# dbking77/ar_slam

Hardware: AMD Instinct MI355X
Metric: LM iterations/sec + ms-to-converged reproj-RMS, 10k-capture synthetic graph (higher is better)
Workload: dtype f64

## Files before the change

### ar_slam_amd/csrc/llt_dag.hip

```cpp
#include "llt_tile.h"
#include "llt_wt.h"

#include <algorithm>
#include <climits>
#include <cmath>

namespace arslam {

namespace {

#ifndef ARSLAM_PIPE_FROM
#define ARSLAM_PIPE_FROM 3
#endif
constexpr int kPipeFrom = ARSLAM_PIPE_FROM;
#ifndef ARSLAM_PIPE_W2
#define ARSLAM_PIPE_W2 1
#endif
constexpr int kPipeW2 = ARSLAM_PIPE_W2;

struct DagArgs {
  double *S;
  int T;
  double *Ld;
  double *ltd;
  const int *rec;
  const int2 *ks_tiles;
  const int *ks;
  int *claimed;
  const int2 *waits;
  int *counters;
  int n_tiles;
  int n_tasks;
  double *part;
  int *split_cnt;
  int *flag;
  int t_begin, t_end;
  int *ticket;
  int *progress;
  unsigned long long *trace;
  int first_store;
  int *started;
  int wg_limit;
};

typedef int int16v __attribute__((ext_vector_type(16)));
struct DagRecV {
  int16v a, b;
  __device__ __forceinline__ int operator[](int i) const { return i < 16 ? a[i] : b[i - 16]; }
};
__device__ __forceinline__ DagRecV load_rec(const int *p) {
  DagRecV r;
  asm volatile("s_load_dwordx16 %0, %2, 0x0\n\ts_load_dwordx16 %1, %2, 0x40\n\ts_waitcnt lgkmcnt(0)"
               : "=s"(r.a), "=s"(r.b)
               : "s"(p)
               : "memory");
  return r;
}
__device__ __forceinline__ DagRecV lds_rec(const int *s) {
  DagRecV r;
#pragma unroll
  for (int i = 0; i < 16; ++i) {
    r.a[i] = __builtin_amdgcn_readfirstlane(s[i]);
    r.b[i] = __builtin_amdgcn_readfirstlane(s[16 + i]);
  }
  return r;
}

enum DagShSlot {
  kShTicket = 0,
  kShBad = 1,
  kShRun = 2,
  kShLast = 3,
  kShClaim = 4,
  kShFetchReq = 6,
  kShFoldCnt = 7,
  kShPipe0 = 8,
  kShThirds = 11,
  kShSolveStep0 = 12,
  kShAkkHalf0 = 16,
  kShTake = 18,
  kShContMet0 = 20,
  kShRec = 24,
  kShInts = kShRec + kDagRecInts
};
static_assert(kShThirds == kShPipe0 + kPfCaller && kShPipe0 + kPfFlags <= kShSolveStep0, "the POTRF pipeline's flags");
static_assert(kShContMet0 + 1 < kShRec && kShInts % 2 == 0, "the slots fit before the record; colx stays 8-byte aligned");

#define DAG_PROGRESS(slot, v)                                                                  \
  do {                                                                                         \
    if (a.progress && tid == 0)                                                                \
      __hip_atomic_store(a.progress + kDagProgressInts * blockIdx.x + (slot), (v), __ATOMIC_RELAXED,          \
                         __HIP_MEMORY_SCOPE_SYSTEM);                                            \
  } while (0)

#ifdef ARSLAM_DAG_SUBSTAMPS
#define DAG_SUBSTAMP(word)                                                                      \
  do {                                                                                          \
    if (a.trace && tid == 0) a.trace[kDagTraceWords * (long)t + (word)] = realtime();           \
  } while (0)
#else
#define DAG_SUBSTAMP(word) do {} while (0)
#endif

__global__ __launch_bounds__(256, kDagWorkgroupsPerCu) void k_factor_dag(DagArgs a) {
  __shared__ __attribute__((aligned(16))) double lds[2 * T64 * LQ + T64 + kLtdSize + kShInts / 2 + T64];
  double *D = lds, *X = lds + T64 * LQ, *inv = X + T64 * LQ, *LTd = inv + T64;
  int *sh = reinterpret_cast<int *>(LTd + kLtdSize);
  int *sh_rec = sh + kShRec;
  double *colx = LTd + kLtdSize + kShInts / 2;
  int *ready = a.counters, *applied = a.counters + a.n_tiles, *ticket = a.ticket;
  int *inflight = a.counters + 2 * a.n_tiles + kDagOffInflight;
  if ((int)blockIdx.x >= a.wg_limit) return;
  if (threadIdx.x == 0) __hip_atomic_fetch_add(a.started, 1, __ATOMIC_RELAXED, __HIP_MEMORY_SCOPE_AGENT);
  int *cu_flag = a.counters + 2 * a.n_tiles + kDagOffCuFlags;
  int cu_key = 0;
  {
    unsigned hw, xcc;
    asm volatile("s_getreg_b32 %0, hwreg(HW_REG_HW_ID)" : "=s"(hw));
    asm volatile("s_getreg_b32 %0, hwreg(HW_REG_XCC_ID)" : "=s"(xcc));
    cu_key = (int)(((xcc & 7u) << 8) | ((hw >> 8) & 0xffu));
  }
  int next = -1, prev_k = -1;
  bool next_met = false;
  bool fast_next = false;
  for (;;) {
    int tid = threadIdx.x;
    asm volatile("" : "+v"(tid));
    const int w = tid >> 6, lane = tid & 63;
    const int r0 = (w >> 1) * 32, c0 = (w & 1) * 32;
    const int li = lane & 15, lk = lane >> 4;
    const bool cont = next >= 0;
    if (!cont) {
      if (tid == 0) sh[kShTicket] = a.t_begin + atomicAdd(ticket, 1);
      __syncthreads();
      next = sh[kShTicket];
      __syncthreads();
    }
    const int t = __builtin_amdgcn_readfirstlane(next);
    const int pk = prev_k;
    const bool premet = cont && next_met;
    const bool fast = cont && fast_next;
    next = -1;
    prev_k = -1;
    next_met = false;
    fast_next = false;
    DAG_PROGRESS(kProgTicket, t);
    DAG_PROGRESS(kProgPhase, 1);
    if (t >= a.t_end) break;
    const DagRecV r = cont ? lds_rec(sh_rec) : load_rec(a.rec + (long)t * kDagRecInts);
    const int4 task = make_int4(r[kRecType], r[kRecY], r[kRecZ], r[kRecW]);
    DAG_PROGRESS(kProgType, task.x);
    if (a.trace && tid == 0) { a.trace[kDagTraceWords * (long)t + kTrDraw] = realtime(); a.trace[kDagTraceWords * (long)t + kTrWg] = blockIdx.x; }
    const int2 sub = make_int2(r[kRecSub], r[kRecLate]);
    if (w == 0) {
      int3 unmet;
      bool expired = false;
      const bool ok =
          premet || dag_wait(a.counters, a.waits, r[kRecWait0], sub.y, a.flag, lane, task.x != 2, &unmet, &expired);
      if (lane == 0) {
        if (!ok) dag_fault(a.flag, a.counters, a.n_tiles, ticket, 1, t, unmet, expired);
        sh[kShRun] = (cont || r[kRecMaxdep] < 0 || atomicCAS(a.claimed + t, 0, 1) == 0) ? 1 : 0;
      }
    }
    if (!fast) {
      __syncthreads();
      if (!sh[kShRun]) continue;
    }
    DAG_PROGRESS(kProgPhase, 2);
    if (a.trace && tid == 0) a.trace[kDagTraceWords * (long)t + kTrMet] = realtime();
    if (task.x != 2) __builtin_amdgcn_s_setprio(3);
    if (task.x == 0) {
      const int k = task.y;
      const int c = sub.x >= 0 ? r[kRecCont] : -1;
      const int apf_tile = sub.x >= 0 ? r[kRecContAkk] : -1;
      const bool apf = apf_tile >= 0;
      const double *apf_src = a.S + (long)max(apf_tile, 0) * (T64 * T64);
      bool ap_met = false;
      int c_rec = 0;
      int2 c_wait = make_int2(0, 0);
      dbl2 apv[16];
#pragma unroll
      for (int u = 0; u < 16; ++u) apv[u] = dbl2{0.0, 0.0};
      bool ap_ok = false;
      if (tid == 0)
        __hip_atomic_store(cu_flag + cu_key, 1, __ATOMIC_RELAXED, __HIP_MEMORY_SCOPE_AGENT);
      const int4 fit = make_int4(0, r[kRecQ0], r[kRecQ1], 0);
      const bool akk_in_d = cont && sh[kShAkkHalf0] && sh[kShAkkHalf0 + 1];
      const bool fold_in = task.z >= 0 && fit.z - fit.y == 1;
      if (fold_in) {
        const double *Akk = a.S + (long)task.w * (T64 * T64);
        if (cont && r[kRecFoldK0] == pk) {
          if (!akk_in_d) load_tile_wt(Akk, D, tid);
        } else load_two_tiles_wt(Akk, D, a.S + (long)r[kRecFoldTile0] * (T64 * T64), X, tid);
      } else if (task.z >= 0) {
        const int4 it = fit;
        dbl4 acc[4] = {{0, 0, 0, 0}, {0, 0, 0, 0}, {0, 0, 0, 0}, {0, 0, 0, 0}};
        double akk[16];
        {
          const double *Akk = a.S + (long)task.w * (T64 * T64);
#pragma unroll
          for (int q = 0; q < 4; ++q) {
            const int rb = r0 + (q >> 1) * 16, cb = c0 + (q & 1) * 16;
#pragma unroll
            for (int reg = 0; reg < 4; ++reg) akk[4 * q + reg] = ld_wt(Akk + (rb + lk + 4 * reg) * T64 + cb + li);
          }
        }
        for (int q = it.y; q < it.z; ++q) {
          if (cont && a.ks[q] == pk) {
            gemm64_nt(X, X, tid, acc);
            continue;
          }
          if (q > it.y) __syncthreads();
          load_tile_wt(a.S + (long)a.ks_tiles[q].x * (T64 * T64), D, tid);
          __syncthreads();
          gemm64_nt(D, D, tid, acc);
        }
        __syncthreads();
#pragma unroll
        for (int q = 0; q < 4; ++q) {
          const int rb = r0 + (q >> 1) * 16, cb = c0 + (q & 1) * 16;
#pragma unroll
          for (int reg = 0; reg < 4; ++reg) D[(rb + lk + 4 * reg) * LQ + cb + li] = akk[4 * q + reg] - acc[q][reg];
        }
      } else {
        load_tile_wt(a.S + (long)task.w * (T64 * T64), D, tid);
      }
      if (!fast) __syncthreads();
      if (a.trace && tid == 0) a.trace[kDagTraceWords * (long)t + kTrLoaded] = realtime();
      const double *pf_src = sub.x >= 0 ? a.S + (long)sub.x * (T64 * T64) : nullptr;
      const int pw0 = sub.y, pw1 = r[kRecWait1];
      const int2 pw_wait = (sub.x >= 0 && pw0 + lane < pw1) ? a.waits[pw0 + lane] : make_int2(0, 0);
      if (tid == 0 && !fast) {
        sh[kShFetchReq] = 0;
        sh[kShSolveStep0] = sh[kShSolveStep0 + 1] = sh[kShSolveStep0 + 2] = sh[kShSolveStep0 + 3] = 0;
        sh[kShTake] = 0;
      }
      bool third_done = false;
      int sdone = 0;
      const bool ok = blocked_potrf64_async(D, inv, LTd, sh + kShBad, sh + kShPipe0, tid, colx, [&](int p, int wv, int ln) {
        auto fetch_third = [&]() {
        auto poll = [&]() {
          if (!pf_src || pw1 - pw0 > 64) return false;
          const int q = pw0 + ln;
          const int got = q < pw1 ? ld_acquire_relaxed(a.counters + pw_wait.x) : 0;
          return __builtin_amdgcn_ballot_w64(q < pw1 && got < pw_wait.y) == 0;
        };
        int lnl = ln;
        asm volatile("" : "+v"(lnl));
        if (p == 0) {
          if (wv == 1 && poll() && ln == 0) *as_lds(sh + kShFetchReq) = -1;
          return;
        }
        if (third_done || lds_get(sh + kShThirds) >= 3) return;
        const int req = lds_get(sh + kShFetchReq);
        bool take = req != 0 && req < p;
        if (req == 0) {
          if (p < 3) {
            if (wv == 1 && poll() && ln == 0) *as_lds(sh + kShFetchReq) = p;
          } else {
            if (!pf_src || pw1 - pw0 > 64) {
              take = false;
            } else if (wv == 1) {
              take = poll();
              lds_set(sh + kShTake, take ? 1 : 2);
            } else {
              lds_wait(sh + kShTake, 1);
              take = lds_get(sh + kShTake) == 1;
            }
          }
        }
        if (take) {
          const int e0 = (wv - 1) * 683, e1 = min(wv * 683, 2048);
          const double *p11[11];
          dbl2 v[11];
#pragma unroll
          for (int u = 0; u < 11; ++u) p11[u] = pf_src + 2 * min(e0 + u * 64 + lnl, e1 - 1);
          ld_wt16x11(p11, v);
#pragma unroll
          for (int u = 0; u < 11; ++u) {
            const int e = e0 + u * 64 + ln, r = e >> 5, c2 = (e & 31) * 2;
            if (e < e1) *reinterpret_cast<dbl2 *>(X + r * LQ + c2) = v[u];
          }
          third_done = true;
          lds_add(sh + kShThirds, ln);
        }
        };
        int c_got = 0;
        bool c_mine = false;
        if (p == 3 && c >= 0 && wv >= 2 && r[kRecContLate] - r[kRecContWait0] <= 64) {
          const int q = r[kRecContWait0] + ln;
          c_mine = q < r[kRecContLate] && c_wait.x != sub.x;
          if (c_mine) c_got = ld_acquire_relaxed(a.counters + c_wait.x);
        }
        fetch_third();
        if (c >= 0 && wv >= 2) {
          const int cw0 = r[kRecContWait0], cw1 = r[kRecContLate];
          if (p == 1 && wv == 3 && ln < kDagRecInts) c_rec = a.rec[(long)c * kDagRecInts + ln];
          if (p == 2) {
            if (wv == 3 && ln < kDagRecInts) sh_rec[ln] = c_rec;
            const int q = cw0 + ln;
            if (q < cw1) c_wait = a.waits[q];
          }
          if (p == 3) {
            const bool met = cw1 - cw0 <= 64 && __builtin_amdgcn_ballot_w64(c_mine && c_got < c_wait.y) == 0;
            if (ln == 0) sh[kShContMet0 + wv - 2] = met ? 1 : 0;
            ap_met = met && apf;
          }
        }
        if (p == 3 && third_done && sdone < 3) lds_wait(sh + kShThirds, 3);
        if (kPipeFrom <= 3 && pf_src && p >= kPipeFrom && sdone < p && lds_get(sh + kShThirds) >= 3) {
          __builtin_amdgcn_fence(__ATOMIC_ACQUIRE, "workgroup");
          for (int st = sdone; st < p; ++st) {
            trsm_step(X, D, LTd, wv - 1, st, ln);
            if (wv == kPipeW2) trsm_step(X, D, LTd, 3, st, ln);
          }
          sdone = p;
          if (ln == 0) {
            sh[kShSolveStep0 + wv - 1] = sdone;
            if (wv == kPipeW2) sh[kShSolveStep0 + 3] = sdone;
          }
        }
      }, X, fold_in, sh + kShFoldCnt);
      const bool keep_flag = sub.x >= 0 && sh[kShThirds] >= 3;
      if (tid == 0 && !keep_flag)
        __hip_atomic_store(cu_flag + cu_key, 0, __ATOMIC_RELAXED, __HIP_MEMORY_SCOPE_AGENT);
      if (a.trace && tid == 0) a.trace[kDagTraceWords * (long)t + kTrFactored] = realtime();
      if (!ok && tid == 0) {
        int first = 0;
        while (first < T64 && D[first * LQ + first] > 0.0) ++first;
        atomicCAS(a.flag, 0, 1 + k * T64 + first);
      }
      double *ltd_g = a.ltd + (long)k * kLtdSize;
      store_tile_wt(a.Ld + (long)k * T64 * T64, D, tid, true);
      for (int e = tid; e < kLtdSize / 2; e += 256)
        st_wt16(ltd_g + 2 * e, *reinterpret_cast<const dbl2 *>(LTd + 2 * e));
      dag_release(tid);
      if (tid == 0) __hip_atomic_fetch_add(ready + task.w, 1, __ATOMIC_RELAXED, __HIP_MEMORY_SCOPE_AGENT);
      if (a.trace && tid == 0) a.trace[kDagTraceWords * (long)t + kTrPublished] = realtime();
      if (sub.x >= 0) {
        const bool pref = sh[kShThirds] >= 3;
        if (!pref) {
          if (w == 0) {
            int3 unmet;
            bool expired = false;
            const bool ok2 = dag_wait(a.counters, a.waits, sub.y, r[kRecWait1], a.flag, lane, true, &unmet, &expired);
            if (!ok2 && lane == 0) dag_fault(a.flag, a.counters, a.n_tiles, ticket, 3, t, unmet, expired);
          }
          __syncthreads();
        }
        double *Ct = a.S + (long)sub.x * (T64 * T64);
        int tk_seen = 0, infl_old = 0, started_seen = 0;
        if (c >= 0 && tid == 0) {
          tk_seen = ld_acquire_relaxed(ticket);
          started_seen = ld_acquire_relaxed(a.started);
          infl_old = atomicAdd(inflight, 1);
        }
        if (!pref) load_tile_wt(Ct, X, tid);
        if (ap_met) {
          int t2 = tid - 128;
          asm volatile("" : "+v"(t2));
          ld_wt16x16_issue(apf_src, t2, apv);
          ap_ok = true;
        }
        __syncthreads();
        DAG_SUBSTAMP(kTrSolveTop);
        const int s0 = pref ? sh[kShSolveStep0 + w] : 0;
        for (int st = s0; st < 2; ++st) trsm_step(X, D, LTd, w, st, lane);
        const bool want = c >= 0 && tid == 0 && a.t_begin + tk_seen > r[kRecContMaxdep] && infl_old < started_seen / 2;
#ifdef ARSLAM_DAG_SUBSTAMPS
        if (a.trace && tid == 0) asm volatile("" ::"v"(tk_seen), "v"(started_seen), "v"(infl_old));
#endif
        DAG_SUBSTAMP(kTrWantKnown);
        int cas_old = 1;
        if (want) cas_old = atomicCAS(a.claimed + c, 0, 1);
        for (int st = max(s0, 2); st < 4; ++st) trsm_step(X, D, LTd, w, st, lane);
        store_elems_wt<64, 512>(Ct, X, 512 * w, lane, false);
        if (keep_flag && tid == 0)
          __hip_atomic_store(cu_flag + cu_key, 0, __ATOMIC_RELAXED, __HIP_MEMORY_SCOPE_AGENT);
        __syncthreads();
        DAG_SUBSTAMP(kTrSolved);
        if (w >= 2) {
          if (ap_ok) {
            ld_wt16x16_wait(apv);
            const int t2 = tid - 128;
#pragma unroll
            for (int u = 0; u < 16; ++u) {
              const int e = u * 128 + t2, row = e >> 5, c2 = (e & 31) * 2;
              *reinterpret_cast<dbl2 *>(D + row * LQ + c2) = apv[u];
            }
          }
          if (lane == 0) sh[kShAkkHalf0 + w - 2] = ap_ok ? 1 : 0;
        }
        if (tid == 0) {
          const int claim = want && cas_old == 0 ? c : -1;
          if (c >= 0 && claim < 0) atomicSub(inflight, 1);
          sh[kShClaim] = claim;
        }
        asm volatile("s_waitcnt vmcnt(0)" ::: "memory");
        __syncthreads();
        DAG_SUBSTAMP(kTrAcked);
        if (tid == 0) __hip_atomic_fetch_add(ready + sub.x, 1, __ATOMIC_RELAXED, __HIP_MEMORY_SCOPE_AGENT);
        if (a.trace && tid == 0) {
          a.trace[kDagTraceWords * (long)t + kTrSubPublished] = realtime();
          const unsigned long long fl = (premet ? 1 : 0) | (akk_in_d ? 2 : 0) | (pref ? 4 : 0) |
                                        (sh[kShContMet0] && sh[kShContMet0 + 1] ? 8 : 0) | (sh[kShClaim] >= 0 ? 16 : 0);
          a.trace[kDagTraceWords * (long)t + kTrWg] = blockIdx.x | (fl << 32);
        }
        __syncthreads();
        next = sh[kShClaim];
        next_met = next >= 0 && sh[kShContMet0] && sh[kShContMet0 + 1];
        if (next >= 0) prev_k = k;
      } else if (r[kRecInv] > 0) {
        blocked_trinv64(D, LTd, X, tid);
        __syncthreads();
        double *Xg = a.Ld + ((long)a.T + k) * T64 * T64;
#pragma unroll
        for (int m = 0; m < 16; ++m) {
          const int e = m * 256 + tid, row = e >> 6, col = e & 63;
          Xg[e] = (row >= col) ? X[col * LQ + row] : 0.0;
        }
      }
    } else if (task.x == 3) {
      const int k = task.y;
      load_tiles_ltd_wt(a.Ld + (long)k * T64 * T64, D, nullptr, nullptr, a.ltd + (long)k * kLtdSize, LTd, tid);
      __syncthreads();
      blocked_trinv64(D, LTd, X, tid);
      __syncthreads();
      double *Xg = a.Ld + ((long)a.T + k) * T64 * T64;
#pragma unroll 4
      for (int m = 0; m < 16; ++m) {
        const int e = m * 256 + tid, r = e >> 6, c = e & 63;
        Xg[e] = (r >= c) ? X[c * LQ + r] : 0.0;
      }
    } else if (task.x == 1) {
      const int k = task.z;
      double *Ct = a.S + (long)task.w * (T64 * T64);
      load_tiles_ltd_wt(Ct, X, a.Ld + (long)k * T64 * T64, D, a.ltd + (long)k * kLtdSize, LTd, tid);
      __syncthreads();
      if (a.trace && tid == 0) a.trace[kDagTraceWords * (long)t + kTrLoaded] = realtime();
      blocked_trsm64(X, D, inv, LTd, tid);
      if (a.trace && tid == 0) a.trace[kDagTraceWords * (long)t + kTrFactored] = realtime();
      store_tile_wt(Ct, X, tid, false);
      dag_release(tid);
      if (tid == 0) __hip_atomic_fetch_add(ready + task.w, 1, __ATOMIC_RELAXED, __HIP_MEMORY_SCOPE_AGENT);
    } else {
      const int4 it = make_int4(0, r[kRecQ0], r[kRecQ1], r[kRecSid]);
      const int ti = r[kRecTi], tj = r[kRecTj], sid = it.w;
      dbl4 acc[4] = {{0, 0, 0, 0}, {0, 0, 0, 0}, {0, 0, 0, 0}, {0, 0, 0, 0}};
      double *C = a.S + (long)task.w * (T64 * T64);
      double cv[16];
      bool c_pre = false;
      if (task.z == 0 && task.w >= a.first_store) {
#pragma unroll
        for (int u = 0; u < 16; ++u) cv[u] = 0.0;
        c_pre = true;
      }
      for (int q = it.y; q < it.z; ++q) {
        const int2 kt = q == it.y ? make_int2(r[kRecTile0I], r[kRecTile0J]) : a.ks_tiles[q];
        if (q > it.y) __syncthreads();
        {
          if (tid == 0) {
            for (int spin = 0; spin < 256 &&
                               __hip_atomic_load(cu_flag + cu_key, __ATOMIC_RELAXED, __HIP_MEMORY_SCOPE_AGENT);
                 ++spin)
              __builtin_amdgcn_s_sleep(8);
          }
          __syncthreads();
        }
        if (q == it.y && sid < 0 && tid == 0)
          sh[kShLast] = (task.z == 0 || ld_acquire_relaxed(applied + task.w) >= task.z) ? 1 : 0;
        if (ti != tj)
          load_two_tiles_wt(a.S + (long)kt.x * (T64 * T64), D, a.S + (long)kt.y * (T64 * T64), X, tid);
        else
          load_tile_wt(a.S + (long)kt.x * (T64 * T64), D, tid);
        __syncthreads();
        const bool c_issue = q == it.z - 1 && sid < 0 && sh[kShLast] && !c_pre;
        if (c_issue) {
#pragma unroll
          for (int u = 0; u < 4; ++u) {
            const int rb = r0 + (u >> 1) * 16, cb = c0 + (u & 1) * 16;
#pragma unroll
            for (int reg = 0; reg < 4; ++reg) cv[4 * u + reg] = ld_wt(C + (rb + lk + 4 * reg) * T64 + cb + li);
          }
          c_pre = true;
        }
        gemm64_nt(D, ti != tj ? X : D, tid, acc);
      }
      bool apply = true;
      if (sid >= 0) {
        const int2 sp = make_int2(r[kRecSplitN], r[kRecSplitP]);
        double *mine = a.part + (long)(sp.y + (sid & 255)) * 4096;
#pragma unroll
        for (int q = 0; q < 4; ++q)
#pragma unroll
          for (int reg = 0; reg < 4; ++reg) st_wt(mine + (4 * q + reg) * 256 + tid, acc[q][reg]);
        dag_release(tid);
        if (tid == 0) {
          const int old = __hip_atomic_fetch_add(a.split_cnt + (sid >> 8), 1, __ATOMIC_RELAXED,
                                                 __HIP_MEMORY_SCOPE_AGENT);
          sh[kShLast] = old == sp.x - 1;
        }
        __syncthreads();
        apply = sh[kShLast] != 0;
        if (apply) {
#pragma unroll
          for (int q = 0; q < 4; ++q) acc[q] = dbl4{0, 0, 0, 0};
          for (int c = 0; c < sp.x; ++c) {
            const double *pc = a.part + (long)(sp.y + c) * 4096;
            double v[16];
            const double *p8[16];
#pragma unroll
            for (int u = 0; u < 16; ++u) p8[u] = pc + u * 256 + tid;
            ld_wt8x8(p8, v);
            ld_wt8x8(p8 + 8, v + 8);
#pragma unroll
            for (int q = 0; q < 4; ++q)
#pragma unroll
              for (int reg = 0; reg < 4; ++reg) acc[q][reg] += v[4 * q + reg];
          }
        }
      }
      DAG_PROGRESS(kProgPhase, 3);
      if (apply && !c_pre) {
        if (tid == 0) {
          long spins = 0;
          int seen;
          WaitTimer tm;
          while ((seen = ld_acquire_relaxed(applied + task.w)) < task.z) {
            __builtin_amdgcn_s_sleep(kPollSleep);
            const bool exp = tm.expired(++spins);
            if (exp || (((spins & 255) == 0) && ld_acquire_relaxed(a.flag) < 0)) {
              dag_fault(a.flag, a.counters, a.n_tiles, ticket, 2, t, make_int3(a.n_tiles + task.w, seen, task.z), exp);
              break;
            }
          }
        }
        __syncthreads();
#pragma unroll
        for (int q = 0; q < 4; ++q) {
          const int rb = r0 + (q >> 1) * 16, cb = c0 + (q & 1) * 16;
#pragma unroll
          for (int reg = 0; reg < 4; ++reg) cv[4 * q + reg] = ld_wt(C + (rb + lk + 4 * reg) * T64 + cb + li);
        }
      }
      if (apply) {
#pragma unroll
        for (int q = 0; q < 4; ++q) {
          const int rb = r0 + (q >> 1) * 16, cb = c0 + (q & 1) * 16;
#pragma unroll
          for (int reg = 0; reg < 4; ++reg)
            st_wt(C + (rb + lk + 4 * reg) * T64 + cb + li, cv[4 * q + reg] - acc[q][reg]);
        }
        dag_release(tid);
        if (tid == 0) __hip_atomic_fetch_add(applied + task.w, 1, __ATOMIC_RELAXED, __HIP_MEMORY_SCOPE_AGENT);
      }
    }
    DAG_PROGRESS(kProgPhase, 4);
    if (cont && tid == 0) atomicSub(inflight, 1);
    __builtin_amdgcn_s_setprio(0);
    if (a.trace && tid == 0) a.trace[kDagTraceWords * (long)t + kTrEnd] = realtime();
  }
  {
    const int tid = threadIdx.x;
    DAG_PROGRESS(kProgPhase, 9);
  }
}

__device__ __forceinline__ void bs_issue_lik(const double *__restrict__ S, int tile, int w, int lane,
                                             double (&lv)[16]) {
  const double *Lik = S + (long)tile * (T64 * T64);
#pragma unroll
  for (int m = 0; m < 16; ++m) lv[m] = Lik[(w + 4 * m) * T64 + lane];
}

__global__ __launch_bounds__(256) void k_bsolve_dag(const double *__restrict__ S, const int *__restrict__ tid_map,
                                                    int T, const double *__restrict__ Ld, long nR,
                                                    const int *__restrict__ cols, const int2 *__restrict__ gather,
                                                    const int *__restrict__ gtile, const int *__restrict__ gbeg,
                                                    int ncols, double *yF, int *counters, int *flag) {
  __shared__ double red[4][T64];
  __shared__ double ys[T64];
  enum { kBsTicket, kBsOk, kBsSlots };
  __shared__ int sh[kBsSlots];
  if (*flag) return;
  const int tid = threadIdx.x, w = tid >> 6, lane = tid & 63;
  int *ticket = counters + T;
  const double *Xinv = Ld + (long)T * T64 * T64;
  const long kr = nR / T64;
  for (;;) {
    if (tid == 0) sh[kBsTicket] = atomicAdd(ticket, 1);
    __syncthreads();
    const int b = __builtin_amdgcn_readfirstlane(sh[kBsTicket]);
    if (b >= ncols) break;
    const int k = cols[b];
    const int g0 = gbeg[b], g1 = gbeg[b + 1];
    const long row0 = (long)k * T64;
    const double *X = Xinv + (long)k * T64 * T64;
    double xv[16];
#pragma unroll
    for (int rr = 0; rr < 16; ++rr) xv[rr] = X[(16 * w + rr) * T64 + lane];
    double z = 0.0;
    if (w == 0 && row0 + lane < nR) {
      if (k == kr) z = Ld[kr * T64 * T64 + (nR - kr * T64) * T64 + lane];
      else z = tile_ptr(S, tid_map, T, (int)kr, k)[(nR - kr * T64) * T64 + lane];
    }
    double acc = 0.0;
    double lvA[16], lvB[16];
    int g = g1 - 1, i_cur = 0, i_nxt = 0, t_nxt = 0;
    if (g >= g0) {
      i_cur = gather[g].x;
      bs_issue_lik(S, gtile[g], w, lane, lvA);
      const int gn = max(g - 1, g0);
      i_nxt = gather[gn].x;
      t_nxt = gtile[gn];
    }
    auto item = [&](double (&lv)[16], double (&lvn)[16]) -> bool {
      const long ri = (long)i_cur * T64;
      double yv = 0.0;
      bool mine = w == 0 && ri + lane < nR;
      if (mine) yv = ld_wt(yF + ri + lane);
      asm volatile("" ::: "memory");
      if (g > g0) bs_issue_lik(S, t_nxt, w, lane, lvn);
      const int gnn = max(g - 2, g0);
      const int i_nn = gather[gnn].x, t_nn = gtile[gnn];
      if (w == 0) {
        bool ok = true;
        long spins = 0;
        WaitTimer tm;
        for (;;) {
// ... 168 lines not shown
```

### ar_slam_amd/csrc/llt_plan.h

```cpp
#pragma once
#include <hip/hip_runtime.h>
#include <algorithm>
#include <climits>
#include <cstdint>
#include <string>
#include <vector>

#include "host_structure.h"

namespace arslam {
constexpr int kCuFlags = 2048;
constexpr int kDagOffTicket0 = 0;
constexpr int kDagOffInflight = 1;
constexpr int kDagOffCuFlags = 2;
constexpr int kDagOffTicket1 = 2 + kCuFlags;
constexpr int kDagOffFault = 3 + kCuFlags;
enum DagFaultField {
  kFaultTicket = 0,
  kFaultKind = 1,
  kFaultCounter = 2,
  kFaultSeen = 3,
  kFaultNeed = 4,
  kFaultDrawn = 5,
  kFaultInflight = 6,
  kFaultBlock = 7,
  kFaultFirstStuck = 8,
  kDagFaultSlots = 9
};
constexpr int kDagOffStarted0 = kDagOffFault + kDagFaultSlots;
constexpr int kDagOffStarted1 = kDagOffStarted0 + 1;
constexpr int kDagCounterExtra = kDagOffStarted1 + 1;
constexpr int kDagWorkgroupsPerCu = 2;

enum DagRecField {
  kRecType = 0, kRecY, kRecZ, kRecW,
  kRecSub, kRecLate, kRecWait0, kRecWait1,
  kRecCont, kRecContAkk, kRecMaxdep,
  kRecContMaxdep, kRecContWait0, kRecContLate,
  kRecInv,
  kRecQ0 = 16, kRecQ1,
  kRecFoldK0, kRecFoldTile0,
  kRecSid = 18, kRecTi, kRecTj,
  kRecSplitN, kRecSplitP,
  kRecTile0I, kRecTile0J,
  kDagRecInts = 32
};

enum DagTraceWord {
  kTrDraw = 0,
  kTrMet = 1,
  kTrEnd = 2,
  kTrWg = 3,
  kTrLoaded = 4,
  kTrFactored = 5,
  kTrPublished = 6,
  kTrSubPublished = 7,
  kTrSolveTop = 8,
  kTrWantKnown = 9,
  kTrSolved = 10,
  kTrAcked = 11,
  kDagTraceWords = 12
};
constexpr int kDagTraceFileWords = 8;
constexpr int kDagTraceSubWords = kDagTraceWords - kDagTraceFileWords;
enum DagProgressSlot {
  kProgTicket = 0,
  kProgPhase = 1,
  kProgType = 2,
  kDagProgressInts = 4
};

struct LltPlan {
  char *arena = nullptr;
  size_t arena_bytes = 0;
  int T = 0;
  long lda = 0;
  int nlev = 0;
  int2 *panel = nullptr;
  int2 *upd_targets = nullptr;
  int *upd_kstart = nullptr;
  int *upd_ks = nullptr;
  int4 *upd_items = nullptr;
  int2 *upd_split = nullptr;
  int *upd_cnt = nullptr;
  double *upd_part = nullptr;
  long n_split = 0, n_part = 0;
  std::vector<int> h_item_off;
  int *bs_cols = nullptr;
  int2 *bs_gather = nullptr;
  int *bs_gbeg = nullptr;
  int *bs_gtile = nullptr;
  double *bs_part = nullptr;
  int *bs_counters = nullptr;
  int *tile_id = nullptr;
  std::vector<int> h_tile_id;
  long n_tiles = 0;
  long n_assembled = 0;
  bool fill_first_ok = false;
  int n_phases = 1;
  long phase_split = 0;
  long n_top_tiles = 0;
  std::vector<int> h_col_class;
  std::vector<int> h_dag_phase;
  signed char *tile_class = nullptr;
  double *ldiag = nullptr;
  std::vector<int> h_panel_off;
  std::vector<int> h_upd_off;
  std::vector<int> h_bs_off;
  std::vector<int> h_bsg_off;
  std::vector<double> h_upd_flops;
  std::vector<int2> h_dag_sub;
  int *dag_claimed = nullptr;
  std::vector<int> h_dag_cont, h_dag_maxdep, h_dag_cont_akk;
  int root_inv_col = -1;
  int *dag_rec = nullptr;
  int2 *dag_ks_tiles = nullptr;
  std::vector<int> h_dag_rec;
  std::vector<int2> h_dag_ks_tiles;
  int2 *dag_waits = nullptr;
  int *dag_counters = nullptr;
  long n_dag_tasks = 0;
  std::vector<int4> h_dag_tasks;
  std::vector<int> h_dag_wait_off;
  std::vector<int2> h_dag_waits;
  std::vector<int2> h_panel, h_targets, h_gather, h_split;
  std::vector<int> h_kstart, h_ks, h_bcols, h_gbeg, h_gtile;
  std::vector<int4> h_items;
  double total_upd_flops = 0.0;
  double total_factor_flops = 0.0;
  long total_upd_tiles = 0;
};

void llt_plan_symbolic(LltPlan &plan, int T, long lda, std::vector<uint8_t> &pattern,
                       const std::vector<int> *col_class = nullptr);
struct RankSplit {
  std::vector<int> col_owner;
  std::vector<int> cap_owner;
  int n_top_cols = 0;
  int n_active = 0;
  double top_work = 0.0, max_rank_work = 0.0, total_work = 0.0;
  std::vector<int> col_class(int rank) const {
    std::vector<int> c(col_owner.size());
    for (size_t k = 0; k < c.size(); ++k) c[k] = col_owner[k] < 0 ? 1 : (col_owner[k] == rank ? 0 : 2);
    return c;
  }
};
RankSplit rank_split(const HostProblem &h, const ReducedLayout &L, int nranks);
bool dag_check(const LltPlan &plan);
bool dag_simulate(const LltPlan &plan, int n_workers, unsigned seed, int policy = 0, int n_started = -1);
constexpr int kDagSimPolicies = 4;
constexpr int kDagSimNoCap = 16;
constexpr int kDagSimGridCap = 32;
int dag_simulate_all(const LltPlan &plan);
std::string dag_fault_detail(const LltPlan &plan, const int *rec);
void llt_plan_upload(LltPlan &plan, hipStream_t s);
void llt_plan_build(LltPlan &plan, int T, long lda, std::vector<uint8_t> &pattern, hipStream_t s,
                    const std::vector<int> *col_class = nullptr);
void llt_plan_free(LltPlan &plan);
void llt_plan_reset(LltPlan &plan);

struct LaunchTiming {
  hipEvent_t *ev = nullptr;
  int cap = 0;
  int used = 0;
  double flops = 0.0;
};

void launch_dense_llt(const LltPlan &P, double *S, int *flag, hipStream_t s,
                      LaunchTiming *timing = nullptr);
void launch_dense_back_solve(const LltPlan &P, const double *S, long nR, double *z, double *yF,
                             const int *flag, hipStream_t s);
void set_dag_workgroup_limit(int k);
inline int dag_launch_grid(long n_tasks, int n_workgroups) {
  return (int)std::min<long>(n_workgroups, std::max<long>(std::min<long>(64, n_tasks), n_tasks / 4));
}
void launch_dense_llt_dag(const LltPlan &P, double *S, int *flag, hipStream_t s, int n_workgroups,
                          int *progress = nullptr, unsigned long long *trace = nullptr, bool reset = true,
                          int phase = -1, long first_store = LONG_MAX);
void launch_dense_back_solve_dag(const LltPlan &P, const double *S, long nR, double *yF, int *flag,
                                 hipStream_t s, int n_workgroups, bool reset = true);
constexpr unsigned long long kYSentinel = 0x7ff47ff47ff47ff4ull;
struct LmDiagArgs {
  long n;
  const double *scale, *colnorm;
  double dmin, dmax;
  double *diag;
  double *ysent = nullptr;
  long nys = 0;
};
void launch_exec_reset(const LltPlan &P, int *flag, hipStream_t s, const LmDiagArgs *ld = nullptr);
struct ExecReset {
  int *flag = nullptr;
  int *a = nullptr, *b = nullptr, *c = nullptr, *d = nullptr;
  long na = 0, nb = 0, nc = 0, nd = 0;
  double *ysent = nullptr;
  long nys = 0;
  __host__ __device__ long n() const { return na + nb + nc + nd > nys ? na + nb + nc + nd : nys; }
};
ExecReset exec_reset_args(const LltPlan &P, int *flag, double *ysent, long nys);
__device__ __forceinline__ void exec_reset_elem(const ExecReset &r, long e) {
  if (e < r.nys) r.ysent[e] = __longlong_as_double((long long)kYSentinel);
  if (e < r.na) r.a[e] = 0;
  else if (e < r.na + r.nb) r.b[e - r.na] = 0;
  else if (e < r.na + r.nb + r.nc) r.c[e - r.na - r.nb] = 0;
  else if (e < r.na + r.nb + r.nc + r.nd) r.d[e - r.na - r.nb - r.nc] = 0;
  if (e == 0 && r.flag) *r.flag = 0;
}
void launch_zero_tiles(const LltPlan &P, double *S, hipStream_t s);
void launch_scatter_diag(const LltPlan &P, double *S, hipStream_t s);

}
```

### ar_slam_amd/csrc/llt_tile.h

```cpp
#pragma once

#include "llt_plan.h"
#include "lm_problem.h"

#include <utility>

namespace arslam {

namespace {

typedef double dbl4 __attribute__((ext_vector_type(4)));
typedef double dbl2 __attribute__((ext_vector_type(2)));

constexpr int T64 = kTile;

#ifdef ARSLAM_STAMPS
__device__ unsigned long long g_stamps[64];
#define STAMP(id)                                                                       \
  do {                                                                                  \
    __builtin_amdgcn_sched_barrier(0);                                                  \
    unsigned long long _t;                                                              \
    asm volatile("s_memtime %0\n\ts_waitcnt lgkmcnt(0)" : "=s"(_t)::"memory");        \
    if (blockIdx.x == 0 && threadIdx.x == 0) g_stamps[id] = _t;                         \
    __builtin_amdgcn_sched_barrier(0);                                                  \
  } while (0)
#else
#define STAMP(id) do {} while (0)
#endif

constexpr int LM = 66;
constexpr int LQ = 66;
constexpr int LI = 18;
constexpr int kLtdSize = 4 * 16 * LI;

__device__ __forceinline__ double *tile_ptr(double *S, const int *tid, int T, int i, int j) {
  return S + (long)tid[(long)i * T + j] * (T64 * T64);
}
__device__ __forceinline__ const double *tile_ptr(const double *S, const int *tid, int T, int i, int j) {
  return S + (long)tid[(long)i * T + j] * (T64 * T64);
}

__device__ __forceinline__ void load_tile_wg(const double *__restrict__ g, long lda, double *lds,
                                             int tid) {
  dbl2 v[8];
#pragma unroll
  for (int q = 0; q < 8; ++q) {
    const int e = q * 256 + tid, r = e >> 5, c2 = (e & 31) * 2;
    v[q] = *reinterpret_cast<const dbl2 *>(g + (long)r * lda + c2);
  }
#pragma unroll
  for (int q = 0; q < 8; ++q) {
    const int e = q * 256 + tid, r = e >> 5, c2 = (e & 31) * 2;
    *reinterpret_cast<dbl2 *>(lds + r * LQ + c2) = v[q];
  }
}

__device__ __forceinline__ void store_tile_wg(double *__restrict__ g, long lda, const double *lds,
                                              int tid, bool lower_only) {
#pragma unroll
  for (int q = 0; q < 8; ++q) {
    const int e = q * 256 + tid, r = e >> 5, c2 = (e & 31) * 2;
    dbl2 v = *reinterpret_cast<const dbl2 *>(lds + r * LQ + c2);
    if (lower_only) {
      if (c2 > r) v.x = 0.0;
      if (c2 + 1 > r) v.y = 0.0;
    }
    *reinterpret_cast<dbl2 *>(g + (long)r * lda + c2) = v;
  }
}

__device__ __forceinline__ double bcast16(double v, int l) {
  switch (l) {
    case 0: return __builtin_amdgcn_mov_dpp(v, 0x150, 0xf, 0xf, false);
    case 1: return __builtin_amdgcn_mov_dpp(v, 0x151, 0xf, 0xf, false);
    case 2: return __builtin_amdgcn_mov_dpp(v, 0x152, 0xf, 0xf, false);
    case 3: return __builtin_amdgcn_mov_dpp(v, 0x153, 0xf, 0xf, false);
    case 4: return __builtin_amdgcn_mov_dpp(v, 0x154, 0xf, 0xf, false);
    case 5: return __builtin_amdgcn_mov_dpp(v, 0x155, 0xf, 0xf, false);
    case 6: return __builtin_amdgcn_mov_dpp(v, 0x156, 0xf, 0xf, false);
    case 7: return __builtin_amdgcn_mov_dpp(v, 0x157, 0xf, 0xf, false);
    case 8: return __builtin_amdgcn_mov_dpp(v, 0x158, 0xf, 0xf, false);
    case 9: return __builtin_amdgcn_mov_dpp(v, 0x159, 0xf, 0xf, false);
    case 10: return __builtin_amdgcn_mov_dpp(v, 0x15a, 0xf, 0xf, false);
    case 11: return __builtin_amdgcn_mov_dpp(v, 0x15b, 0xf, 0xf, false);
    case 12: return __builtin_amdgcn_mov_dpp(v, 0x15c, 0xf, 0xf, false);
    case 13: return __builtin_amdgcn_mov_dpp(v, 0x15d, 0xf, 0xf, false);
    case 14: return __builtin_amdgcn_mov_dpp(v, 0x15e, 0xf, 0xf, false);
    case 15: return __builtin_amdgcn_mov_dpp(v, 0x15f, 0xf, 0xf, false);
    default: return v;
  }
}

__device__ __forceinline__ void wave_gemm16_sub(double *C, const double *A, const double *B, int K,
                                                int lane) {
  const int li = lane & 15, lk = lane >> 4;
  double c[4];
#pragma unroll
  for (int reg = 0; reg < 4; ++reg) c[reg] = C[(lk + 4 * reg) * LQ + li];
  dbl4 acc = {0, 0, 0, 0};
  for (int k4 = 0; k4 < K; k4 += 4) {
    const double a = A[li * LQ + k4 + lk];
    const double b = B[li * LQ + k4 + lk];
    acc = __builtin_amdgcn_mfma_f64_16x16x4f64(a, b, acc, 0, 0, 0);
  }
#pragma unroll
  for (int reg = 0; reg < 4; ++reg) C[(lk + 4 * reg) * LQ + li] = c[reg] - acc[reg];
}


__device__ __forceinline__ void wave_apply_inv16(double *C, const double *Linv, int lane) {
  const int li = lane & 15, lk = lane >> 4;
  double a[4];
#pragma unroll
  for (int q = 0; q < 4; ++q) a[q] = C[li * LQ + 4 * q + lk];
  __builtin_amdgcn_wave_barrier();
  dbl4 acc = {0, 0, 0, 0};
#pragma unroll
  for (int q = 0; q < 4; ++q)
    acc = __builtin_amdgcn_mfma_f64_16x16x4f64(a[q], Linv[li * LI + 4 * q + lk], acc, 0, 0, 0);
#pragma unroll
  for (int reg = 0; reg < 4; ++reg) C[(lk + 4 * reg) * LQ + li] = acc[reg];
}

template <int j>
__device__ __forceinline__ void elim_step(double &x0, double &x1, double &x2, double &x3, double &R, double nf,
                                          double y0, double y1, double y2, double y3, double rj) {
  constexpr unsigned m = (0xffffu << (j + 1)) & 0xffffu;
  constexpr unsigned BL = m | (m << 16);
  constexpr int g = j >> 2;
  constexpr unsigned CL = g == 0 ? m : g == 1 ? (m << 16) : 0u;
  constexpr unsigned CH = g == 2 ? m : g == 3 ? (m << 16) : 0u;
  unsigned sl, sh;
#define ARSLAM_ELIM_ASM(XS)                                                                   \
  asm volatile("s_mov_b32 %[sl], exec_lo\n\t"                                                 \
               "s_mov_b32 %[sh], exec_hi\n\t"                                                 \
               "s_and_b32 exec_lo, %[sl], %[bl]\n\t"                                          \
               "s_and_b32 exec_hi, %[sh], %[bl]\n\t"                                          \
               "v_fma_f64 %[x0], %[nf], %[y0], %[x0]\n\t"                                     \
               "v_fma_f64 %[x1], %[nf], %[y1], %[x1]\n\t"                                     \
               "v_fma_f64 %[x2], %[nf], %[y2], %[x2]\n\t"                                     \
               "v_fma_f64 %[x3], %[nf], %[y3], %[x3]\n\t"                                     \
               "v_fma_f64 %[R], %[nf], %[rj], %[R]\n\t"                                       \
               "s_and_b32 exec_lo, %[sl], %[cl]\n\t"                                          \
               "s_and_b32 exec_hi, %[sh], %[ch]\n\t"                                          \
               "v_mov_b64 %[" XS "], %[nf]\n\t"                                               \
               "s_mov_b32 exec_lo, %[sl]\n\t"                                                 \
               "s_mov_b32 exec_hi, %[sh]\n\t"                                                 \
               "s_nop 4"           \
               : [x0] "+v"(x0), [x1] "+v"(x1), [x2] "+v"(x2), [x3] "+v"(x3), [R] "+v"(R),      \
                 [sl] "=&s"(sl), [sh] "=&s"(sh)                                                \
               : [nf] "v"(nf), [y0] "v"(y0), [y1] "v"(y1), [y2] "v"(y2), [y3] "v"(y3),          \
                 [rj] "v"(rj), [bl] "i"(BL), [cl] "i"(CL), [ch] "i"(CH))
  switch (j & 3) {
    case 0: ARSLAM_ELIM_ASM("x0"); break;
    case 1: ARSLAM_ELIM_ASM("x1"); break;
    case 2: ARSLAM_ELIM_ASM("x2"); break;
    default: ARSLAM_ELIM_ASM("x3"); break;
  }
#undef ARSLAM_ELIM_ASM
}

template <int j>
__device__ __forceinline__ void diag16_pivot(double (&x)[4], double &R, double &R2, double *colx, int lane) {
  const int i = lane & 15;
  const double ajj = bcast16(R, j);
  const double r0 = __builtin_amdgcn_rcp(ajj);
  const double e = __builtin_fma(-ajj, r0, 1.0);
  const double nf0 = -R * r0;
  const double pe = __builtin_fma(e, e, e);
  const double nf = __builtin_fma(nf0, pe, nf0);
  double xj[4];
#pragma unroll
  for (int q = 0; q < 4; ++q) xj[q] = bcast16(x[q], j);
  const double rj = j + 1 < 16 ? bcast16(R2, j) : 0.0;
  R = R2;
  elim_step<j>(x[0], x[1], x[2], x[3], R, nf, xj[0], xj[1], xj[2], xj[3], rj);
  if (j + 2 < 16) {
    colx[lane] = x[(j + 2) & 3];
    R2 = colx[16 * ((j + 2) >> 2) + i];
  }
}

template <int... J>
__device__ __forceinline__ void diag16_pivots(double (&x)[4], double &R, double &R2, double *colx, int lane,
                                              std::integer_sequence<int, J...>) {
  (diag16_pivot<J>(x, R, R2, colx, lane), ...);
}

__device__ __forceinline__ void diag16(double *D, int b0, double *inv, double *Li, int *bad, int lane,
                                       double *colx) {
  __builtin_amdgcn_fence(__ATOMIC_RELEASE, "wavefront");
  __builtin_amdgcn_wave_barrier();
  __builtin_amdgcn_fence(__ATOMIC_ACQUIRE, "wavefront");
  const int g = lane >> 4, i = lane & 15;
  double x[4];
#pragma unroll
  for (int q = 0; q < 4; ++q) {
    const int c = 4 * g + q;
    x[q] = c <= i ? D[(b0 + i) * LQ + b0 + c] : D[(b0 + c) * LQ + b0 + i];
  }
  double R = D[(b0 + i) * LQ + b0];
  double R2 = i >= 1 ? D[(b0 + i) * LQ + b0 + 1] : D[(b0 + 1) * LQ + b0];
  diag16_pivots(x, R, R2, colx, lane, std::make_integer_sequence<int, 16>{});
  __builtin_amdgcn_wave_barrier();
  if (g == (i >> 2)) colx[i] = (i & 3) == 0 ? x[0] : (i & 3) == 1 ? x[1] : (i & 3) == 2 ? x[2] : x[3];
  __builtin_amdgcn_fence(__ATOMIC_RELEASE, "wavefront");
  __builtin_amdgcn_wave_barrier();
  __builtin_amdgcn_fence(__ATOMIC_ACQUIRE, "wavefront");
  const double piv = colx[i];
  if (!(piv > 0.0)) *bad = 1;
  const double d = sqrt(piv), rd = 1.0 / d;
#pragma unroll
  for (int q = 0; q < 4; ++q) {
    const int c = 4 * g + q;
    D[(b0 + c) * LQ + b0 + i] = c > i ? x[q] * rd : (c == i ? d : 0.0);
    Li[i * LI + c] = c < i ? x[q] * rd : (c == i ? rd : 0.0);
  }
  if (g == 0) inv[b0 + i] = rd;
}

template <class Idle>
__device__ bool blocked_potrf64_idle(double *D, double *inv, double *LTd, int *bad, int tid, double *colx,
                                     Idle &&idle, const double *F = nullptr) {
  const int w = tid >> 6, lane = tid & 63;
  if (tid == 0) *bad = 0;
  __syncthreads();
  for (int p = 0; p < 4; ++p) {
    const int b0 = 16 * p;
    STAMP(10 + 4 * p);
    if (w == 0) {
      if (p == 0 && F) wave_gemm16_sub(D, F, F, 64, lane);
      if (p > 0) wave_gemm16_sub(D + b0 * LQ + b0, D + b0 * LQ + b0 - 16, D + b0 * LQ + b0 - 16, 16, lane);
      diag16(D, b0, inv, LTd + p * 16 * LI, bad, lane, colx);
    } else if (p == 0) {
      if (F) {
        for (int t = w; t < 10; t += 3) {
          int I = 0;
          while ((I + 1) * (I + 2) / 2 <= t) ++I;
          const int C = t - I * (I + 1) / 2;
          wave_gemm16_sub(D + 16 * I * LQ + 16 * C, F + 16 * I * LQ, F + 16 * C * LQ, 64, lane);
        }
      }
      idle(0, w, lane);
    } else {
      const int m = 4 - p, ntl = m * (m + 1) / 2;
      for (int t = w; t < ntl; t += 3) {
        int I = 0;
        while ((I + 1) * (I + 2) / 2 <= t) ++I;
        const int C = t - I * (I + 1) / 2;
        const int bi = 16 * (p + I), bc = 16 * (p + C);
        wave_gemm16_sub(D + bi * LQ + bc, D + bi * LQ + b0 - 16, D + bc * LQ + b0 - 16, 16, lane);
      }
      idle(p, w, lane);
    }
    __syncthreads();
    STAMP(11 + 4 * p);
    if (p < 3) {
      if (w < 3 - p) wave_apply_inv16(D + (b0 + 16 + 16 * w) * LQ + b0, LTd + p * 16 * LI, lane);
      __syncthreads();
    }
    STAMP(12 + 4 * p);
    STAMP(13 + 4 * p);
  }
  return *bad == 0;
}

typedef __attribute__((address_space(3))) volatile int lds_vint;
__device__ __forceinline__ lds_vint *as_lds(const int *f) { return (lds_vint *)(f); }
__device__ __forceinline__ void lds_set(int *f, int v) {
  __builtin_amdgcn_fence(__ATOMIC_RELEASE, "workgroup");
  *as_lds(f) = v;
}
__device__ __forceinline__ void lds_add(int *f, int lane) {
  __builtin_amdgcn_fence(__ATOMIC_RELEASE, "workgroup");
  if (lane == 0) __hip_atomic_fetch_add(f, 1, __ATOMIC_RELAXED, __HIP_MEMORY_SCOPE_WORKGROUP);
}
__device__ __forceinline__ int lds_get(const int *f) { return *as_lds(f); }
__device__ __forceinline__ void lds_wait(const int *f, int v) {
  while (*as_lds(f) < v) __builtin_amdgcn_s_sleep(0);
  __builtin_amdgcn_fence(__ATOMIC_ACQUIRE, "workgroup");
}

enum PotrfFlag {
  kPfPanel = 0,
  kPfApplied = 1,
  kPfRound = 2,
  kPfCaller = 3,
  kPfFlags = 4
};
template <class Idle>
__device__ bool blocked_potrf64_async(double *D, double *inv, double *LTd, int *bad, int *fl, int tid,
                                      double *colx, Idle &&idle, const double *F = nullptr, bool fold = false,
                                      int *fcnt = nullptr) {
  const int w = tid >> 6, lane = tid & 63;
  const bool early = fold && fcnt;
  if (tid == 0) {
    *bad = 0;
    fl[kPfPanel] = fl[kPfApplied] = fl[kPfRound] = fl[kPfCaller] = 0;
    if (fcnt) *fcnt = 0;
  }
  __syncthreads();
  if (w == 0) {
    STAMP(30);
    for (int p = 0; p < 4; ++p) {
      const int b0 = 16 * p;
      if (p == 0 && fold) wave_gemm16_sub(D, F, F, 64, lane);
      STAMP(31 + 6 * p);
      STAMP(32 + 6 * p);
      diag16(D, b0, inv, LTd + p * 16 * LI, bad, lane, colx);
      STAMP(33 + 6 * p);
      if (p < 3) {
        if (p == 0 && early) lds_wait(fcnt, 2);
        else lds_wait(fl + kPfRound, 3 * (p + 1));
        STAMP(34 + 6 * p);
        const int li = lane & 15, lk = lane >> 4;
        double *Cb = D + (b0 + 16) * LQ + b0, *Cd = Cb + 16;
        const double *Linv = LTd + p * 16 * LI;
        double a[4], cd[4];
#pragma unroll
        for (int q = 0; q < 4; ++q) a[q] = Cb[li * LQ + 4 * q + lk];
#pragma unroll
        for (int reg = 0; reg < 4; ++reg) cd[reg] = Cd[(lk + 4 * reg) * LQ + li];
        __builtin_amdgcn_wave_barrier();
        dbl4 y = {0, 0, 0, 0};
#pragma unroll
        for (int q = 0; q < 4; ++q) y = __builtin_amdgcn_mfma_f64_16x16x4f64(Linv[li * LI + 4 * q + lk], a[q], y, 0, 0, 0);
#pragma unroll
        for (int reg = 0; reg < 4; ++reg) Cb[li * LQ + lk + 4 * reg] = y[reg];
        lds_set(fl + kPfPanel, p + 1);
        STAMP(35 + 6 * p);
        dbl4 g = {0, 0, 0, 0};
#pragma unroll
        for (int reg = 0; reg < 4; ++reg) g = __builtin_amdgcn_mfma_f64_16x16x4f64(y[reg], y[reg], g, 0, 0, 0);
#pragma unroll
        for (int reg = 0; reg < 4; ++reg) Cd[(lk + 4 * reg) * LQ + li] = cd[reg] - g[reg];
      }
    }
  } else {
    if (fold) {
      for (int t = w; t < 10; t += 3) {
        int I = 0;
        while ((I + 1) * (I + 2) / 2 <= t) ++I;
        const int C = t - I * (I + 1) / 2;
        wave_gemm16_sub(D + 16 * I * LQ + 16 * C, F + 16 * I * LQ, F + 16 * C * LQ, 64, lane);
        if (early && t <= 2) lds_add(fcnt, lane);
      }
    }
    idle(0, w, lane);
    lds_add(fl + kPfRound, lane);
    for (int p = 0; p < 3; ++p) {
      const int b0 = 16 * p;
      if (p == 0 && early) lds_wait(fl + kPfRound, 3);
      lds_wait(fl + kPfPanel, p + 1);
      if (w < 3 - p - 1 + 1 && p + 1 + w <= 3)
        wave_apply_inv16(D + (b0 + 16 * (1 + w)) * LQ + b0, LTd + p * 16 * LI, lane);
      lds_add(fl + kPfApplied, lane);
      lds_wait(fl + kPfApplied, 3 * (p + 1));
      const int m = 3 - p, ntl = m * (m + 1) / 2;
      for (int t = w; t < ntl; t += 3) {
        int I = 0;
        while ((I + 1) * (I + 2) / 2 <= t) ++I;
        const int C = t - I * (I + 1) / 2;
        const int bi = 16 * (p + 1 + I), bc = 16 * (p + 1 + C);
        wave_gemm16_sub(D + bi * LQ + bc, D + bi * LQ + b0, D + bc * LQ + b0, 16, lane);
      }
      idle(p + 1, w, lane);
      lds_add(fl + kPfRound, lane);
    }
  }
  __syncthreads();
  return *bad == 0;
}

__device__ __forceinline__ bool blocked_potrf64(double *D, double *inv, double *LTd, int *bad, int tid, double *colx) {
  return blocked_potrf64_idle(D, inv, LTd, bad, tid, colx, [](int, int, int) {});
}

__device__ __forceinline__ void trsm_step(double *X, const double *D, const double *LTd, int rb, int p, int lane) {
  const int b0 = 16 * p;
  if (p > 0) wave_gemm16_sub(X + 16 * rb * LQ + b0, X + 16 * rb * LQ, D + b0 * LQ, b0, lane);
  __builtin_amdgcn_fence(__ATOMIC_RELEASE, "wavefront");
  __builtin_amdgcn_wave_barrier();
  __builtin_amdgcn_fence(__ATOMIC_ACQUIRE, "wavefront");
  wave_apply_inv16(X + 16 * rb * LQ + b0, LTd + p * 16 * LI, lane);
  __builtin_amdgcn_fence(__ATOMIC_RELEASE, "wavefront");
  __builtin_amdgcn_wave_barrier();
  __builtin_amdgcn_fence(__ATOMIC_ACQUIRE, "wavefront");
}

__device__ __forceinline__ void blocked_trsm64(double *X, const double *D, const double *inv, const double *LTd,
                               int tid) {
  const int w = tid >> 6, lane = tid & 63;
  for (int p = 0; p < 4; ++p) trsm_step(X, D, LTd, w, p, lane);
  __syncthreads();
}

__device__ __forceinline__ void blocked_trinv64(const double *D, const double *LTd, double *XT, int tid) {
  const int q = tid >> 6, lane = tid & 63;
  const int li = lane & 15, lk = lane >> 4;
  const double *Lq = LTd + q * 16 * LI;
#pragma unroll
  for (int e = 0; e < 4; ++e) {
    const int idx = lane + 64 * e, i = idx >> 4, j = idx & 15;
    XT[(16 * q + j) * LQ + 16 * q + i] = (j <= i) ? Lq[i * LI + j] : 0.0;
  }
  double *scr = XT + (q == 0 ? 48 : 16 * q) * LQ;
  __builtin_amdgcn_fence(__ATOMIC_RELEASE, "wavefront");
  __builtin_amdgcn_wave_barrier();
  __builtin_amdgcn_fence(__ATOMIC_ACQUIRE, "wavefront");
  for (int p = q + 1; p < 4; ++p) {
    dbl4 acc = {0, 0, 0, 0};
    for (int r = q; r < p; ++r)
#pragma unroll
      for (int k4 = 0; k4 < 4; ++k4) {
        const double a = D[(16 * p + li) * LQ + 16 * r + 4 * k4 + lk];
        const double b = XT[(16 * q + li) * LQ + 16 * r + 4 * k4 + lk];
        acc = __builtin_amdgcn_mfma_f64_16x16x4f64(a, b, acc, 0, 0, 0);
      }
#pragma unroll
    for (int reg = 0; reg < 4; ++reg) scr[li * LQ + lk + 4 * reg] = acc[reg];
    __builtin_amdgcn_fence(__ATOMIC_RELEASE, "wavefront");
    __builtin_amdgcn_wave_barrier();
    __builtin_amdgcn_fence(__ATOMIC_ACQUIRE, "wavefront");
    dbl4 x = {0, 0, 0, 0};
    const double *Lp = LTd + p * 16 * LI;
#pragma unroll
    for (int k4 = 0; k4 < 4; ++k4)
      x = __builtin_amdgcn_mfma_f64_16x16x4f64(Lp[li * LI + 4 * k4 + lk], scr[li * LQ + 4 * k4 + lk], x, 0, 0, 0);
#pragma unroll
    for (int reg = 0; reg < 4; ++reg) XT[(16 * q + li) * LQ + 16 * p + lk + 4 * reg] = -x[reg];
    __builtin_amdgcn_fence(__ATOMIC_RELEASE, "wavefront");
    __builtin_amdgcn_wave_barrier();
    __builtin_amdgcn_fence(__ATOMIC_ACQUIRE, "wavefront");
  }
}

__device__ __forceinline__ void gemm64_nt(const double *sA, const double *sB, int tid, dbl4 acc[4]) {
  const int w = tid >> 6, lane = tid & 63;
  const int r0 = (w >> 1) * 32, c0 = (w & 1) * 32;
  const int li = lane & 15, lk = lane >> 4;
#pragma unroll 4
  for (int kk = 0; kk < T64 / 4; ++kk) {
    const int kc = kk * 4 + lk;
    const double a0 = sA[(r0 + li) * LQ + kc];
    const double a1 = sA[(r0 + 16 + li) * LQ + kc];
    const double b0 = sB[(c0 + li) * LQ + kc];
    const double b1 = sB[(c0 + 16 + li) * LQ + kc];
    acc[0] = __builtin_amdgcn_mfma_f64_16x16x4f64(a0, b0, acc[0], 0, 0, 0);
    acc[1] = __builtin_amdgcn_mfma_f64_16x16x4f64(a0, b1, acc[1], 0, 0, 0);
    acc[2] = __builtin_amdgcn_mfma_f64_16x16x4f64(a1, b0, acc[2], 0, 0, 0);
    acc[3] = __builtin_amdgcn_mfma_f64_16x16x4f64(a1, b1, acc[3], 0, 0, 0);
  }
}

__device__ __forceinline__ void acc_pos(int tid, int q, int reg, int &row, int &col) {
  const int w = tid >> 6, lane = tid & 63;
  row = (w >> 1) * 32 + (q >> 1) * 16 + (lane >> 4) + 4 * reg;
  col = (w & 1) * 32 + (q & 1) * 16 + (lane & 15);
}

}

}
```

Baseline: 1178.

## Signal round completion before idle work and move row-block-3 solve to wave 0

Helper waves in the async 64x64 Cholesky now bump the round counter before running their idle callback rather than after. This lets wave 0 start the next panel without waiting on prefetch or solve work done in the idle hook. The fourth row-block of the fused triangular solve (rb=3), previously handled by wave 1, now runs on wave 0 after it finishes its panels, through a new idle(4,0) call. Optional timestamp instrumentation is added behind a compile flag. The risk is that wave 0 carries extra serial solve work at the tail, and signalling early could expose ordering problems if the idle hook touches tiles that later rounds read.

```diff
diff --git a/ar_slam_amd/csrc/llt_dag.hip b/ar_slam_amd/csrc/llt_dag.hip
--- a/ar_slam_amd/csrc/llt_dag.hip
+++ b/ar_slam_amd/csrc/llt_dag.hip
@@ -14,7 +14,7 @@
 #endif
 constexpr int kPipeFrom = ARSLAM_PIPE_FROM;
 #ifndef ARSLAM_PIPE_W2
-#define ARSLAM_PIPE_W2 1
+#define ARSLAM_PIPE_W2 0
 #endif
 constexpr int kPipeW2 = ARSLAM_PIPE_W2;
 
@@ -237,7 +237,20 @@
       }
       bool third_done = false;
       int sdone = 0;
+#ifdef ARSLAM_DAG_SUBSTAMPS
+      unsigned long long *const ws = a.trace ? a.trace + kDagTraceWords * (long)t + kTrPfStamp0 : nullptr;
+#else
+      unsigned long long *const ws = nullptr;
+#endif
       const bool ok = blocked_potrf64_async(D, inv, LTd, sh + kShBad, sh + kShPipe0, tid, colx, [&](int p, int wv, int ln) {
+        if (wv == 0) {
+          if (kPipeW2 == 0 && kPipeFrom <= 3 && pf_src && lds_get(sh + kShThirds) >= 3) {
+            __builtin_amdgcn_fence(__ATOMIC_ACQUIRE, "workgroup");
+            for (int st = 0; st < 3; ++st) trsm_step(X, D, LTd, 3, st, ln);
+            if (ln == 0) sh[kShSolveStep0 + 3] = 3;
+          }
+          return;
+        }
         auto fetch_third = [&]() {
         auto poll = [&]() {
           if (!pf_src || pw1 - pw0 > 64) return false;
@@ -320,11 +333,21 @@
             if (wv == kPipeW2) sh[kShSolveStep0 + 3] = sdone;
           }
         }
-      }, X, fold_in, sh + kShFoldCnt);
+#ifdef ARSLAM_DAG_SUBSTAMPS
+        if (p == 3 && ln == 0) *as_lds(sh + (wv == 1 ? 19 : 20 + wv)) = (int)realtime();
+#endif
+      }, X, fold_in, sh + kShFoldCnt, ws);
       const bool keep_flag = sub.x >= 0 && sh[kShThirds] >= 3;
       if (tid == 0 && !keep_flag)
         __hip_atomic_store(cu_flag + cu_key, 0, __ATOMIC_RELAXED, __HIP_MEMORY_SCOPE_AGENT);
       if (a.trace && tid == 0) a.trace[kDagTraceWords * (long)t + kTrFactored] = realtime();
+#ifdef ARSLAM_DAG_SUBSTAMPS
+      if (a.trace && tid == 0) {
+        a.trace[kDagTraceWords * (long)t + kTrPfStamp0 + kPsIdle1] = (unsigned)sh[19];
+        a.trace[kDagTraceWords * (long)t + kTrPfStamp0 + kPsIdle1 + 1] = (unsigned)sh[22];
+        a.trace[kDagTraceWords * (long)t + kTrPfStamp0 + kPsIdle1 + 2] = (unsigned)sh[23];
+      }
+#endif
       if (!ok && tid == 0) {
         int first = 0;
         while (first < T64 && D[first * LQ + first] > 0.0) ++first;
diff --git a/ar_slam_amd/csrc/llt_plan.h b/ar_slam_amd/csrc/llt_plan.h
--- a/ar_slam_amd/csrc/llt_plan.h
+++ b/ar_slam_amd/csrc/llt_plan.h
@@ -59,7 +59,12 @@
   kTrWantKnown = 9,
   kTrSolved = 10,
   kTrAcked = 11,
+#ifdef ARSLAM_DAG_SUBSTAMPS
+  kTrPfStamp0 = 12,
+  kDagTraceWords = 22
+#else
   kDagTraceWords = 12
+#endif
 };
 constexpr int kDagTraceFileWords = 8;
 constexpr int kDagTraceSubWords = kDagTraceWords - kDagTraceFileWords;
diff --git a/ar_slam_amd/csrc/llt_tile.h b/ar_slam_amd/csrc/llt_tile.h
--- a/ar_slam_amd/csrc/llt_tile.h
+++ b/ar_slam_amd/csrc/llt_tile.h
@@ -288,10 +288,34 @@
   kPfCaller = 3,
   kPfFlags = 4
 };
+#ifndef ARSLAM_PF_COUNT_FIRST
+#define ARSLAM_PF_COUNT_FIRST 1
+#endif
+constexpr bool kPfCountFirst = ARSLAM_PF_COUNT_FIRST != 0;
+enum PfStamp {
+  kPsWait0 = 0,
+  kPsClose = 6,
+  kPsIdle1 = 7,
+  kPsStamps = 10
+};
+#ifdef ARSLAM_DAG_SUBSTAMPS
+#define PF_WSTAMP(ws, i, lane)                                                                \
+  do {                                                                                        \
+    if (ws) {                                                                                 \
+      __builtin_amdgcn_sched_barrier(0);                                                      \
+      unsigned long long _t;                                                                  \
+      asm volatile("s_memrealtime %0\n\ts_waitcnt lgkmcnt(0)" : "=s"(_t)::"memory");         \
+      if ((lane) == 0) ((__attribute__((address_space(1))) unsigned long long *)(ws))[i] = _t;  \
+      __builtin_amdgcn_sched_barrier(0);                                                      \
+    }                                                                                         \
+  } while (0)
+#else
+#define PF_WSTAMP(ws, i, lane) do {} while (0)
+#endif
 template <class Idle>
 __device__ bool blocked_potrf64_async(double *D, double *inv, double *LTd, int *bad, int *fl, int tid,
                                       double *colx, Idle &&idle, const double *F = nullptr, bool fold = false,
-                                      int *fcnt = nullptr) {
+                                      int *fcnt = nullptr, unsigned long long *ws = nullptr) {
   const int w = tid >> 6, lane = tid & 63;
   const bool early = fold && fcnt;
   if (tid == 0) {
@@ -310,8 +334,10 @@
       diag16(D, b0, inv, LTd + p * 16 * LI, bad, lane, colx);
       STAMP(33 + 6 * p);
       if (p < 3) {
+        PF_WSTAMP(ws, kPsWait0 + 2 * p, lane);
         if (p == 0 && early) lds_wait(fcnt, 2);
         else lds_wait(fl + kPfRound, 3 * (p + 1));
+        PF_WSTAMP(ws, kPsWait0 + 2 * p + 1, lane);
         STAMP(34 + 6 * p);
         const int li = lane & 15, lk = lane >> 4;
         double *Cb = D + (b0 + 16) * LQ + b0, *Cd = Cb + 16;
@@ -336,6 +362,8 @@
         for (int reg = 0; reg < 4; ++reg) Cd[(lk + 4 * reg) * LQ + li] = cd[reg] - g[reg];
       }
     }
+    idle(4, 0, lane);
+    PF_WSTAMP(ws, kPsClose, lane);
   } else {
     if (fold) {
       for (int t = w; t < 10; t += 3) {
@@ -346,8 +374,9 @@
         if (early && t <= 2) lds_add(fcnt, lane);
       }
     }
+    if (kPfCountFirst) lds_add(fl + kPfRound, lane);
     idle(0, w, lane);
-    lds_add(fl + kPfRound, lane);
+    if (!kPfCountFirst) lds_add(fl + kPfRound, lane);
     for (int p = 0; p < 3; ++p) {
       const int b0 = 16 * p;
       if (p == 0 && early) lds_wait(fl + kPfRound, 3);
@@ -364,8 +393,9 @@
         const int bi = 16 * (p + 1 + I), bc = 16 * (p + 1 + C);
         wave_gemm16_sub(D + bi * LQ + bc, D + bi * LQ + b0, D + bc * LQ + b0, 16, lane);
       }
+      if (kPfCountFirst) lds_add(fl + kPfRound, lane);
       idle(p + 1, w, lane);
-      lds_add(fl + kPfRound, lane);
+      if (!kPfCountFirst) lds_add(fl + kPfRound, lane);
     }
   }
   __syncthreads();
```

After: 1206 (median of 6 runs). 2.3% higher.
